# liuyuan-pal/Gen6D

Hardware: NVIDIA H100
Metric: poses/sec end-to-end (128^2 crop, 64 refs, 3 refine iters) (higher is better)
Workload: dtype f32

## Files before the change

### gen6d_b200/_lib.py

```python
import ctypes as C
import os
import re

HERE = os.path.dirname(os.path.abspath(__file__))
LIB_PATH = os.path.join(HERE, 'libgen6d_b200.so')
HEADER_PATH = os.path.join(os.path.dirname(HERE), 'include', 'gen6d_b200.h')

G6D_DET_MAX_SCALES = 8
G6D_GLUE_MAX_OBJECTS = 16
G6D_DET_MAX_INSTANCES = 16
G6D_DET_MAX_PEAK_RADIUS = 3
G6D_ATTENTION_MAX_SMEM_FLOATS = 12288 - 32
G6D_FRAMES_MAX = 1024
G6D_FRAME_RGB, G6D_FRAME_NV12 = 0, 1
G6D_DRAW_MAX_BOXES = 16
PRO_NONE, PRO_AFFINE, PRO_AFFINE_RELU, PRO_CORR = 0, 1, 2, 3
ACT_NONE, ACT_RELU, ACT_LEAKY01 = 0, 1, 2
TC_TF32, TC_F16 = 0, 1
TC_PRENORM, TC_REUSE_IM2COL, TC_FOLD_SPLITS = 1, 4, 32


class ConvDesc(C.Structure):
    _fields_ = [(n, C.c_int) for n in ('B', 'D', 'H', 'W', 'Cin', 'in_cstride', 'in_coff', 'Cout', 'kd', 'kh', 'kw',
                                       'stride', 'pd', 'ph', 'pw', 'Do', 'Ho', 'Wo', 'out_cstride', 'out_coff',
                                       'prologue')] + [('group_rows', C.c_longlong), ('act', C.c_int), ('max_chain_k', C.c_int),
                                                      ('plan_rows', C.c_int)]


class DetMaps(C.Structure):
    _fields_ = [('n_scales', C.c_int), ('rfn', C.c_int), ('hs', C.c_int), ('ws', C.c_int),
                ('map', (C.c_void_p * 3) * G6D_DET_MAX_SCALES),
                ('H', (C.c_int * 3) * G6D_DET_MAX_SCALES), ('W', (C.c_int * 3) * G6D_DET_MAX_SCALES),
                ('mu', C.c_float * 3), ('inv_sigma', C.c_float * 3), ('clip', C.c_float)]

# ... 158 lines not shown
```

### gen6d_b200/csrc/conv_tc.cu

```cuda
#include <cuda_fp16.h>
#include <string.h>

#include "tc_common.cuh"

namespace g6d {

constexpr int TC_BM = 128;
constexpr int TC_PRODUCER_WARPS = 8;
constexpr int TC_CONSUMER_WARPS = 8;
constexpr int TC_THREADS = (TC_PRODUCER_WARPS + TC_CONSUMER_WARPS) * 32;
constexpr int TC_ISSUER = TC_PRODUCER_WARPS * 32;
constexpr int TC_PRODUCER_REGS = 96, TC_CONSUMER_REGS = 160;
static_assert(TC_PRODUCER_WARPS * TC_PRODUCER_REGS + TC_CONSUMER_WARPS * TC_CONSUMER_REGS <= 65536 / 32, "register file of one SM");
constexpr int TC_FOLD_PRODUCER_REGS = 40, TC_FOLD_CONSUMER_REGS = 216;
static_assert(TC_PRODUCER_WARPS * TC_FOLD_PRODUCER_REGS + TC_CONSUMER_WARPS * TC_FOLD_CONSUMER_REGS <= 65536 / 32, "register file of one SM");
static_assert(TC_BM == 64 * (TC_CONSUMER_WARPS / 4), "one 64-row wgmma tile per consumer warpgroup");
constexpr int TC_MAX_K_PER_CHAIN = 2048;

template <int KIND> struct KindCfg;
template <> struct KindCfg<G6D_TC_TF32> {
    static constexpr int BK = 32;
    static constexpr int NV = 1;
    static constexpr float CROSS = 1.f;
};
template <> struct KindCfg<G6D_TC_F16> {
    static constexpr int BK = 64;
    static constexpr int NV = 2;
    static constexpr float CROSS = 1.f / 2048.f;
};
constexpr float F16_LO_SCALE = 2048.f;
constexpr int TC2_RING = 2, FLAT_RING = 3;
// ... 234 lines not shown
                                              int lane) {
    sum_chains<BN, KIND>(acc, cross, n_acc);
    store_tile<BN>(cross, dst0, dst1, n_base, Cout, bias, act, partial, vec2, stats, group, lane);
}

constexpr int TC2_PF_BYTES = 12 * 128;

template <int BN> struct Tc2Cfg {
    static constexpr int A_BYTES = TC_BM * 128;
    static constexpr int B_BYTES = BN * 128;
    static constexpr int STAGE_BYTES = 2 * A_BYTES + 2 * B_BYTES;
    static constexpr int STAGES = (208 * 1024) / STAGE_BYTES > 6 ? 6 : (208 * 1024) / STAGE_BYTES;
    static constexpr int SMEM_BYTES = STAGES * STAGE_BYTES + 1024 + 256;
};

template <int BN> struct Tc2XrCfg {
    static constexpr int BOX_ROWS = 144;
    static constexpr int BOX_BYTES = BOX_ROWS * 128;
    static constexpr int BOXES = 3;
    static constexpr int B_BYTES = BN * 128;
    static constexpr int B_STAGES = 6;
    static constexpr int SMEM_BYTES = BOXES * 2 * BOX_BYTES + B_STAGES * 2 * B_BYTES + 1024 + 256;
};
static_assert(Tc2XrCfg<64>::SMEM_BYTES <= 227 * 1024, "x-reuse rings of BN 64");

struct Tc2Work { int m_tiles, n_tiles, total; };

template <int BN, int KIND, bool FOLD, bool XR>
__global__ void __launch_bounds__(TC_THREADS, 1)
conv_tc2_kernel(const ConvTcP p, const Tc2Work wk, const __grid_constant__ CUtensorMap map_hi,
                const __grid_constant__ CUtensorMap map_lo, const __grid_constant__ CUtensorMap map_a) {
    using Cfg = Tc2Cfg<BN>;
    using XC = Tc2XrCfg<BN>;
    using KC = KindCfg<KIND>;
    constexpr int NPW = TC_PRODUCER_WARPS;
    constexpr int STAGES = Cfg::STAGES;
    constexpr int NMAIN = AccCfg<BN>::NMAIN;
    constexpr int BK = KC::BK, NV = KC::NV;
    constexpr int RSTEP = NPW * 4;
    constexpr int ROWS = TC_BM / RSTEP;
    constexpr int RING = TC2_RING;
    constexpr int PF = TC2_PF_BYTES / 128;
    extern __shared__ uint8_t smem_raw[];
    const uint32_t base = (smem_u32(smem_raw) + 1023u) & ~1023u;
    const uint32_t bar_base = base + STAGES * Cfg::STAGE_BYTES;
    auto a_hi = [&](int s) { return base + s * Cfg::STAGE_BYTES; };
    auto a_lo = [&](int s) { return base + s * Cfg::STAGE_BYTES + Cfg::A_BYTES; };
    auto b_hi = [&](int s) { return base + s * Cfg::STAGE_BYTES + 2 * Cfg::A_BYTES; };
    auto b_lo = [&](int s) { return base + s * Cfg::STAGE_BYTES + 2 * Cfg::A_BYTES + Cfg::B_BYTES; };
    auto full_a = [&](int s) { return bar_base + 8 * s; };
// ... 2 lines not shown
    auto box_hi = [&](int s) { return base + s * 2 * XC::BOX_BYTES; };
    auto box_lo = [&](int s) { return base + s * 2 * XC::BOX_BYTES + XC::BOX_BYTES; };
    const uint32_t xb_base = base + XC::BOXES * 2 * XC::BOX_BYTES;
    auto xb_hi = [&](int s) { return xb_base + s * 2 * XC::B_BYTES; };
    auto xb_lo = [&](int s) { return xb_base + s * 2 * XC::B_BYTES + XC::B_BYTES; };
    const uint32_t xbar = xb_base + XC::B_STAGES * 2 * XC::B_BYTES;
    auto box_full = [&](int s) { return xbar + 8 * s; };
    auto box_empty = [&](int s) { return xbar + 8 * (XC::BOXES + s); };
    auto xb_full = [&](int s) { return xbar + 8 * (2 * XC::BOXES + s); };
    auto xb_empty = [&](int s) { return xbar + 8 * (2 * XC::BOXES + XC::B_STAGES + s); };

    const int warp = threadIdx.x >> 5, lane = threadIdx.x & 31;
    if (XR && threadIdx.x == TC_ISSUER) {
        for (int s = 0; s < XC::BOXES; ++s) {
            mbar_init(box_full(s), 1);
            mbar_init(box_empty(s), TC_CONSUMER_WARPS);
        }
        for (int s = 0; s < XC::B_STAGES; ++s) {
            mbar_init(xb_full(s), 1);
            mbar_init(xb_empty(s), TC_CONSUMER_WARPS);
        }
        fence_barrier_init();
        asm volatile("prefetch.tensormap [%0];" ::"l"(&map_hi) : "memory");
        asm volatile("prefetch.tensormap [%0];" ::"l"(&map_lo) : "memory");
        asm volatile("prefetch.tensormap [%0];" ::"l"(&map_a) : "memory");
    } else if (threadIdx.x == TC_ISSUER) {
        for (int s = 0; s < STAGES; ++s) {
            mbar_init(full_a(s), p.split_in ? 1 : NPW);
            mbar_init(full_b(s), 1);
            mbar_init(empty(s), TC_CONSUMER_WARPS);
        }
        fence_barrier_init();
        asm volatile("prefetch.tensormap [%0];" ::"l"(&map_hi) : "memory");
        asm volatile("prefetch.tensormap [%0];" ::"l"(&map_lo) : "memory");
        if (p.split_in) asm volatile("prefetch.tensormap [%0];" ::"l"(&map_a) : "memory");
    }
    __syncthreads();

    auto decode = [&](int w, int& mt, int& nt, int& sp) {
        nt = w % wk.n_tiles; w /= wk.n_tiles;
        mt = w % wk.m_tiles;
        sp = w / wk.m_tiles;
    };
    auto kblocks_of = [&](int sp) { return min(p.kblocks, sp * p.kb_per_split + p.kb_per_split) - sp * p.kb_per_split; };
    const int chains = FOLD ? p.splits : 1;
    auto chain_of = [&](int j, int& mt, int& nt, int& sp) {
        const int w = blockIdx.x + (j / chains) * gridDim.x;
        if (w >= wk.total) return false;
        decode(w, mt, nt, sp);
        sp += j % chains;
        return true;
    };

    if (warp < NPW) {
        setmaxnreg_dec<FOLD ? TC_FOLD_PRODUCER_REGS : TC_PRODUCER_REGS>();
        if (XR && threadIdx.x == 0) {
            const bool vol = p.D > 1 || p.kd > 1;
            const uint32_t box_tx = 2u * p.xr_rows * 128u;
            int g = 0, gb = 0;
            int mt, nt, sp;
            for (int j = 0; chain_of(j, mt, nt, sp); ++j) {
                const int nkb = kblocks_of(sp);
                int m = mt * TC_BM;
                const int xo = m % p.Wp; m /= p.Wp;
                const int yo = m % p.Ho; m /= p.Ho;
                const int zo = m % p.Do;
                const int b = m / p.Do;
                KbIter pf, k;
                pf.start(p, sp, 0);
                k = pf;
                auto prefetch = [&]() {
                    const int kc = pf.tap(p) * p.Cin + pf.cb * BK;
                    tma_prefetch_2d(&map_hi, kc, nt * BN);
                    tma_prefetch_2d(&map_lo, kc, nt * BN);
                    pf.next(p);
                };
#pragma unroll 1
                for (int i = 0; i < min(nkb, PF - 1); ++i) prefetch();
// ... 10 lines not shown
                        } else {
                            tma_im2col_4d(box_hi(s), &map_a, box_full(s), 2 * BK * k.cb, xo - p.pw, yo - p.ph, b, 0, oy);
                            tma_im2col_4d(box_lo(s), &map_a, box_full(s), 2 * BK * k.cb + BK, xo - p.pw, yo - p.ph, b, 0, oy);
                        }
                        ++gb;
                    }
                    const int s = g % XC::B_STAGES;
                    mbar_wait(xb_empty(s), ((g / XC::B_STAGES) & 1) ^ 1, 1, g);
                    mbar_expect_tx(xb_full(s), 2 * XC::B_BYTES);
                    tma_load_2d(xb_hi(s), &map_hi, xb_full(s), k.tap(p) * p.Cin + k.cb * BK, nt * BN);
                    tma_load_2d(xb_lo(s), &map_lo, xb_full(s), k.tap(p) * p.Cin + k.cb * BK, nt * BN);
                }
            }
            return;
        }
        if (XR || FOLD || p.split_in) {
            if (!XR && threadIdx.x == 0) {
                const bool vol = p.D > 1 || p.kd > 1;
                int g = 0;
                int mt, nt, sp;
                for (int j = 0; chain_of(j, mt, nt, sp); ++j) {
                    const int nkb = kblocks_of(sp);
                    int m = mt * TC_BM;
                    const int xo = m % p.Wo; m /= p.Wo;
                    const int yo = m % p.Ho; m /= p.Ho;
                    const int zo = m % p.Do;
                    const int b = m / p.Do;
                    KbIter pf, k;
                    pf.start(p, sp, 0);
                    k = pf;
                    auto prefetch = [&]() {
                        const int kc = pf.tap(p) * p.Cin + pf.cb * BK;
                        tma_prefetch_2d(&map_hi, kc, nt * BN);
                        tma_prefetch_2d(&map_lo, kc, nt * BN);
                        pf.next(p);
                    };
#pragma unroll 1
                    for (int i = 0; i < min(nkb, PF - 1); ++i) prefetch();
// ... 213 lines not shown
            }
            wgmma_wait<0>();
            if (nkb > 0) release(g - 1);
            }

            sum_chains<BN, KIND>(acc, cross, nkb < NMAIN ? nkb : NMAIN);
            if constexpr (FOLD) {
#pragma unroll
                for (int jj = 0; jj < BN / 2; ++jj) run[jj] = (sp == 0 ? 0.f : run[jj]) + cross[jj];
                if (sp < p.splits - 1) continue;
#pragma unroll
                for (int jj = 0; jj < BN / 2; ++jj) cross[jj] = run[jj];
            }
            const bool partial = p.splits > 1 && !FOLD;
            const int n_base = nt * BN;
            const int m0 = mt * TC_BM + 16 * cw + (lane >> 2), m1 = m0 + 8;
            float* out = partial ? p.ws + (long long)sp * p.M * p.Cout + n_base : p.y + p.oco + n_base;
            const long long ld = partial ? p.Cout : p.ocs;
            const bool vec2 = partial ? (p.Cout & 1) == 0
                                      : ((p.ocs & 1) == 0 && (p.oco & 1) == 0 && (reinterpret_cast<uintptr_t>(p.y) & 7) == 0);
            auto dst = [&](int m) -> float* {
                if constexpr (XR) {
                    if (m >= p.Mp) return nullptr;
                    const int q = m / p.Wp, xp = m - q * p.Wp;
                    return xp < p.Wo ? out + ((long long)q * p.Wo + xp) * ld : nullptr;
                } else {
                    return m < p.M ? out + m * ld : nullptr;
                }
            };
            store_tile<BN>(cross, dst(m0), dst(m1), n_base, p.Cout, p.bias,
                           p.act, partial, vec2, p.stats, (long long)(mt * TC_BM + 16 * cw) / p.stats_rows, lane);
        }
    }
}


__global__ void conv_tc_reduce_kernel(const float* __restrict__ ws, const float* __restrict__ bias,
                                      float* __restrict__ y, int M, int Cout, int splits, int ocs, int oco, int act) {
    const long long i = (long long)blockIdx.x * blockDim.x + threadIdx.x;
    if (i >= (long long)M * Cout) return;
    const int n = (int)(i % Cout);
    const long long m = i / Cout;
    float v = 0.f;
    for (int s = 0; s < splits; ++s) v += ws[(long long)s * M * Cout + i];
    if (bias) v += bias[n];
    y[m * ocs + oco + n] = tc_act(v, act);
}

// ... 221 lines not shown
        splits = (int)(kNumSMs / ctas);
        splits = splits > p.kblocks / min_kb ? p.kblocks / min_kb : splits;
        splits = splits < 1 ? 1 : splits;
    }
    const int nmain = tc_nmain(bn);
    const int chain = d->max_chain_k > 0 ? d->max_chain_k * nmain : (K > TC_MAX_K_PER_CHAIN ? TC_MAX_K_PER_CHAIN * nmain : 0);
    const int max_kb = chain > bk ? chain / bk : 1;
    const int min_splits = chain > 0 ? (p.kblocks + max_kb - 1) / max_kb : 1;
    splits = splits < min_splits ? min_splits : splits;
    splits = splits > 64 ? 64 : splits;
    p.kb_per_split = (p.kblocks + splits - 1) / splits;
    p.splits = (p.kblocks + p.kb_per_split - 1) / p.kb_per_split;
    return G6D_OK;
}

template <int BN, int KIND, bool FOLD, bool XR>
static int launch_tc2(const ConvTcP& p, const CUtensorMap& mh, const CUtensorMap& ml, const CUtensorMap& ma, cudaStream_t st) {
    constexpr int SMEM = XR ? Tc2XrCfg<BN>::SMEM_BYTES : Tc2Cfg<BN>::SMEM_BYTES;
    static bool configured = false;
    if (!configured) {
        cudaError_t e = cudaFuncSetAttribute(conv_tc2_kernel<BN, KIND, FOLD, XR>, cudaFuncAttributeMaxDynamicSharedMemorySize, SMEM);
        if (e != cudaSuccess) { set_error("g6d_conv_tc: cannot opt in to %d B of shared memory: %s", SMEM, cudaGetErrorString(e)); return G6D_ECUDA; }
        configured = true;
    }
    Tc2Work wk;
    wk.m_tiles = ceil_div(XR ? p.Mp : p.M, TC_BM); wk.n_tiles = ceil_div(p.Cout, BN);
    const long long total = (long long)wk.m_tiles * wk.n_tiles * (FOLD ? 1 : p.splits);
    wk.total = (int)total;
    const int grid = total < kNumSMs ? (int)total : kNumSMs;
    conv_tc2_kernel<BN, KIND, FOLD, XR><<<grid, TC_THREADS, SMEM, st>>>(p, wk, mh, ml, ma);
    G6D_CHECK_LAUNCH("g6d_conv_tc");
    return G6D_OK;
}

__global__ void split_tf32_kernel(const float* __restrict__ in, float* __restrict__ hi, float* __restrict__ lo, long long n) {
    const long long i = (long long)blockIdx.x * blockDim.x + threadIdx.x;
    if (i >= n) return;
    const float v = in[i];
    const float h = to_tf32(v);
    hi[i] = h;
    lo[i] = to_tf32(v - h);
}
__device__ __forceinline__ void split_f16_scalar(float v, __half& h, __half& l) {
    uint32_t hh, ll;
    split_f16x2(v, 0.f, hh, ll);
// ... 358 lines not shown
    if (!configured) {
        cudaError_t e = cudaFuncSetAttribute(conv_tcflat_kernel<BN, KIND>, cudaFuncAttributeMaxDynamicSharedMemorySize, 227 * 1024);
        if (e != cudaSuccess) { set_error("g6d_conv_tc(flat): cannot opt in to shared memory: %s", cudaGetErrorString(e)); return G6D_ECUDA; }
        configured = true;
    }
    dim3 grid((unsigned)((long long)p.B * p.Do * p.tiles_per_plane), ceil_div(p.Cout, BN), p.splits);
    conv_tcflat_kernel<BN, KIND><<<grid, TC_THREADS, smem, st>>>(p, mh, ml);
    G6D_CHECK_LAUNCH("g6d_conv_tc(flat)");
    return G6D_OK;
}

struct ConvPlan {
    ConvTcP tc;
    ConvFlatP flat;
    bool use_flat;
    int bn, splits, flat_smem;
    long long split_in_off;
    long long ws_bytes;
};

constexpr double TC_FOLD_SLACK = 0.15;

static bool fold_ok(const ConvPlan& pl) {
    if (pl.use_flat || !pl.tc.split_in || pl.splits < 2) return false;
    const long long T = (long long)ceil_div(pl.tc.M, TC_BM) * ceil_div(pl.tc.Cout, pl.bn), S = pl.splits;
    return (double)(ceil_div(T, kNumSMs) * S) <= (1.0 + TC_FOLD_SLACK) * (double)ceil_div(T * S, kNumSMs);
}

static bool split_input_ok(const g6d_conv_desc* d, int kind, int flags, bool use_flat) {
    if (use_flat || kind != G6D_TC_F16 || (d->prologue != G6D_PRO_NONE && !(flags & G6D_TC_PRENORM)) || d->stride != 1 ||
        d->kd * d->kh * d->kw == 1)
        return false;
    if (!split_input_rank5(d)) return d->kw <= 64 && d->kh <= 64 && d->pw < 64 && d->ph < 64;
    auto corners_ok = [](int k, int pad) { return k <= 16 && pad <= 16 && pad - (k - 1) >= -16 && pad - (k - 1) <= 15; };
    return (flags & G6D_TC_REUSE_IM2COL) && corners_ok(d->kw, d->pw) && corners_ok(d->kh, d->ph) && corners_ok(d->kd, d->pd);
}

static bool xr_ok(const g6d_conv_desc* d, const ConvPlan& pl) {
    if (!pl.tc.split_in || !pl.tc.reuse_order || pl.bn != 64 || d->kw < 2 || d->kw > 17) return false;
    if (split_input_rank5(d) && d->pw > 15) return false;
    return (long long)pl.tc.M / pl.tc.Wo * (pl.tc.Wo + d->kw - 1) < (1ll << 31);
}

static int make_plan(const g6d_conv_desc* d, int kind, int flags, ConvPlan& pl) {
    G6D_REQUIRE((flags & ~(G6D_TC_PRENORM | G6D_TC_REUSE_IM2COL | G6D_TC_FOLD_SPLITS)) == 0, "g6d_conv_tc: bad flags %d", flags);
    const int rc = fill_tc_params(d, kind, pl.tc);
    if (rc != G6D_OK) return rc;
    pl.use_flat = fill_flat_params(d, kind, pl.flat, &pl.flat_smem);
    pl.tc.reuse_order = 0;
    if (pl.use_flat && (flags & G6D_TC_REUSE_IM2COL) && split_input_ok(d, kind, flags, false)) {
        pl.use_flat = false;
        pl.tc.reuse_order = 1;
        pl.tc.kb_per_split = pl.flat.cb_per_split * d->kd * d->kh * d->kw;
        pl.tc.splits = pl.flat.splits;
    }
    pl.bn = tc_block_n(d->Cout);
    pl.splits = pl.use_flat ? pl.flat.splits : pl.tc.splits;
    pl.tc.split_in = split_input_ok(d, kind, flags, pl.use_flat) ? 1 : 0;
    pl.tc.fold = (flags & G6D_TC_FOLD_SPLITS) && fold_ok(pl) ? 1 : 0;
    pl.tc.xr = xr_ok(d, pl) ? 1 : 0;
    if (pl.tc.xr) {
        pl.tc.Wp = pl.tc.Wo + d->kw - 1;
        pl.tc.Mp = (int)((long long)pl.tc.M / pl.tc.Wo * pl.tc.Wp);
        pl.tc.xr_rows = (TC_BM + d->kw - 1 + 7) / 8 * 8;
    }
    const long long partials =
        pl.splits > 1 && !pl.tc.fold ? (long long)pl.splits * pl.tc.M * pl.tc.Cout * (long long)sizeof(float) : 0;
    pl.split_in_off = (partials + 255) / 256 * 256;
    pl.ws_bytes = pl.tc.split_in
                      ? pl.split_in_off + (long long)d->B * d->D * d->H * d->W * d->Cin * 2 * (long long)sizeof(__half)
                      : partials;
    return G6D_OK;
}

static bool stats_ok(const ConvPlan& pl, long long stats_rows) {
    if (stats_rows <= 0 || stats_rows % 32 != 0 || pl.tc.M % stats_rows != 0) return false;
    return !(pl.use_flat || pl.tc.reuse_order) || stats_rows % ((long long)pl.flat.Ho * pl.flat.Wo) == 0;
}

template <class P>
static void bind_tensors(P& p, const float* x, const float* bias, const float* ps, const float* pb, float* y, void* ws,
                         double* stats, long long stats_rows) {
    p.x = x; p.bias = bias; p.ps = ps; p.pb = pb; p.y = y; p.ws = static_cast<float*>(ws);
    p.stats = stats; p.stats_rows = stats ? stats_rows : 1;
}

template <int BN, int KIND>
static int launch_plan(const ConvPlan& pl, const CUtensorMap& mh, const CUtensorMap& ml, const CUtensorMap& ma, cudaStream_t st) {
    if (pl.use_flat) return launch_flat<BN, KIND>(pl.flat, pl.flat_smem, mh, ml, st);
    if constexpr (KIND == G6D_TC_F16) {
        if constexpr (BN == 64)
            if (pl.tc.xr) return pl.tc.fold ? launch_tc2<BN, KIND, true, true>(pl.tc, mh, ml, ma, st)
                                            : launch_tc2<BN, KIND, false, true>(pl.tc, mh, ml, ma, st);
        if (pl.tc.fold) return launch_tc2<BN, KIND, true, false>(pl.tc, mh, ml, ma, st);
    }
    return launch_tc2<BN, KIND, false, false>(pl.tc, mh, ml, ma, st);
}
template <int KIND>
static int dispatch(const ConvPlan& pl, const CUtensorMap& mh, const CUtensorMap& ml, const CUtensorMap& ma, cudaStream_t st) {
    if (pl.bn == 128) return launch_plan<128, KIND>(pl, mh, ml, ma, st);
    if (pl.bn == 64) return launch_plan<64, KIND>(pl, mh, ml, ma, st);
    return launch_plan<32, KIND>(pl, mh, ml, ma, st);
}

}
// ... 36 lines not shown
    ConvPlan pl{};
    const int rc = make_plan(desc, kind, flags, pl);
    if (rc != G6D_OK) return rc;
    out4[0] = pl.use_flat ? 1 : 0;
    out4[1] = pl.bn;
    out4[2] = pl.splits;
    out4[3] = pl.tc.split_in;
    return G6D_OK;
}

extern "C" int g6d_conv_tc_plan_v2(const g6d_conv_desc* desc, int kind, int flags, int* out, int n) {
    G6D_REQUIRE(out != nullptr && n > 0, "g6d_conv_tc_plan_v2: null output");
    ConvPlan pl{};
    const int rc = make_plan(desc, kind, flags, pl);
    if (rc != G6D_OK) return rc;
    const int v[6] = {pl.use_flat ? 1 : 0, pl.bn, pl.splits, pl.tc.split_in, pl.tc.fold, pl.tc.xr};
    for (int i = 0; i < n && i < 6; ++i) out[i] = v[i];
    return G6D_OK;
}

extern "C" int g6d_conv_tc_plan(const g6d_conv_desc* desc, int kind, int* out4) {
    return g6d_conv_tc_plan_ex(desc, kind, 0, out4);
}

extern "C" int g6d_conv_tc_ex(const g6d_conv_desc* desc, const float* x, const void* w_hi, const void* w_lo, int w_rows,
                              int kind, const float* bias, const float* pro_scale, const float* pro_shift, float* y,
                              void* ws, double* stats, long long stats_rows, int flags, g6d_stream_t stream) {
    ConvPlan pl{};
    int rc = make_plan(desc, kind, flags, pl);
    if (rc != G6D_OK) return rc;
    const ConvTcP& p = pl.tc;
    if (stats) G6D_REQUIRE(stats_ok(pl, stats_rows), "g6d_conv_tc: fused statistics need groups of whole 32-row slices / planes (stats_rows %lld)", stats_rows);
// ... 126 lines not shown
```

### gen6d_b200/network/backbone.py

```python
import torch

from .. import ops
from .params import VGG11_BLOCKS

BN_EPS = 1e-5


def pack_vgg(params):
    packed = {}
    f = params.features
    with torch.no_grad():
        for block in VGG11_BLOCKS:
            for slot in block:
                conv, bn = f[slot], f[slot + 1]
                scale = (bn.weight / torch.sqrt(bn.running_var + BN_EPS)).float().contiguous()
                bias = ((conv.bias - bn.running_mean) * scale + bn.bias).float().contiguous()
                packed[slot] = ops.pack_conv(conv.weight, stride=1, pad=1, cout_scale=scale, bias_override=bias)
    return packed


def vgg_pyramid(packed, x, full_res=False):
    outs = []
    fused = not full_res and x.shape[1] % 2 == 0 and x.shape[2] % 2 == 0 and x.shape[3] == 4
    for bi, block in enumerate(VGG11_BLOCKS):
        if bi == 0 and fused:
            outs.append(None)
            x = ops.vgg_first_block(x, packed[block[0]])
            continue
        if bi > 0 and not (bi == 1 and fused):
            x = ops.maxpool2x2(x)
        for slot in block:
            x = ops.conv(x, packed[slot], act=ops.ACT_NONE if slot == 25 else ops.ACT_RELU, reuse_im2col=True,
                         fold_splits=True)
        outs.append(x)
    outs.append(ops.maxpool2x2(x))
    return outs


def vgg_v1(packed, x):
    p = vgg_pyramid(packed, x)
    return p[3], p[4], p[5]


def vgg_v3(packed, x):
    p = vgg_pyramid(packed, x)
    return p[2], p[3], p[4]
```

### gen6d_b200/network/detector.py

```python
from dataclasses import dataclass

import numpy as np
import torch

from .. import ops
from .backbone import pack_vgg, vgg_v1
from .base import Branches, PackedModule
from .params import VGG11BNParams, detector_heads


@dataclass
class DetectorRefs:
    center_feats: list
    kernels: list
    shape: tuple = (120, 120)

    @property
    def rfn(self):
        return self.center_feats[0].shape[0]


class Detector(PackedModule):
    default_cfg = {
        'vgg_score_stats': [[36.264317, 13.151907], [13910.291, 5345.965], [829.70807, 387.98788]],
# ... 64 lines not shown
    def scale_sizes(self, hq, wq):
        out = []
        for s in self.cfg['detection_scales']:
            ht, wt = int(np.round(hq * 2 ** s)), int(np.round(wq * 2 ** s))
            if ht % 32 != 0:
                ht = (ht // 32 + 1) * 32
            if wt % 32 != 0:
                wt = (wt // 32 + 1) * 32
            out.append((ht, wt))
        return out

    def _raw_correlation(self, que01):
        feats = self._features(que01)
        out = []
        for f, pc in zip(feats, self.ref_kernels):
            y = ops.conv(f, pc, reuse_im2col=True, fold_splits=True)
            rows = getattr(pc, 'rows', None)
            out.append(ops.det_corr_rowsum(y, *rows) if rows is not None else y)
        return out

    def _raw_correlation_objects(self, que01, kernels, n_obj, rfn):
        feats = self._features(que01)
        out = []
        for f, pc in zip(feats, kernels):
            y = ops.conv(f, pc, reuse_im2col=True, fold_splits=True)
            k = pc.rows[0] if pc.rows is not None else 1
            m = ops.det_corr_rowsum_objects(y, n_obj, k, rfn)
            out.append(m.reshape(n_obj * m.shape[1], *m.shape[2:]))
        return out

    def _detect_nhwc(self, que01, return_taps=False):
        if self.ref_kernels is None:
            raise RuntimeError('Detector: load_ref_imgs / load_impl must be called first')
        return self._detect_maps(que01, self._raw_correlation, que01.shape[0], self.refs.rfn, return_taps)

    def _detect_objects_nhwc(self, que01, kernels, n_obj, rfn, return_taps=False):
        return self._detect_maps(que01, lambda cur: self._raw_correlation_objects(cur, kernels, n_obj, rfn),
                                 n_obj * que01.shape[0], rfn, return_taps)

    def _detect_maps(self, que01, correlate, rows, rfn, return_taps):
# ... 7 lines not shown
            cur = que01 if (ht, wt) == (hq, wq) else ops.resize_bilinear(que01, ht, wt)
            return correlate(cur)

        maps = [br.run(i, lambda ht=ht, wt=wt: one_scale(ht, wt)) for i, (ht, wt) in enumerate(scales)]
        br.join()
        sizes = [[(r.shape[1], r.shape[2]) for r in raw] for raw in maps]
        feats = ops.det_score_fuse(maps, sizes, rfn, hs, ws, self.cfg['vgg_score_stats'], self.cfg['vgg_score_max'],
                                   p['w1'], p['b1'], p['w2'], p['b2'], rows)
        outs = {}
        heads = ('score_predict', 'scale_predict', 'offset_predict')
        hb = Branches(len(heads))

        def one_head(head):
            x = feats
            for i, pc in enumerate(p[head]):
                x = ops.conv(x, pc, act=ops.ACT_RELU if i < 2 else ops.ACT_NONE, reuse_im2col=True, fold_splits=True)
            return x

        for i, head in enumerate(heads):
            outs[head] = hb.run(i, lambda head=head: one_head(head))
        hb.join()
        if return_taps:
            outs['raw'] = maps
            outs['scores_feats'] = feats
        return outs

    def _detect_u8(self, u8):
        o = self._detect_nhwc(ops.preprocess_u8(u8, out_c=3, imagenet_norm=False))
        out, _ = ops.det_parse(o['score_predict'], o['scale_predict'], o['offset_predict'], self.pool_ratio)
        return out

# ... 35 lines not shown
```

### gen6d_b200/network/refiner.py

```python
import threading
from dataclasses import dataclass, field

import numpy as np
import torch

from .. import ops
from .backbone import pack_vgg, vgg_v3
from .base import Branches, PackedModule, linear_as_conv
from .params import RefineFeatureParams, RefineRegressorParams, RefineVolumeParams

IN_EPS = 1e-5
_UPLOAD_LOCK = threading.Lock()
IM2COL = dict(prenorm=True, reuse_im2col=True, fold_splits=True)


@dataclass
class RefinerRefs:
    database: object
    ids: list
    dev: dict = field(default_factory=dict)
    src: dict = field(default_factory=dict)


class VolumeRefiner(PackedModule):
    default_cfg = {'refiner_sample_num': 32}

    def __init__(self, cfg):
        self.cfg = {**self.default_cfg, **cfg}
# ... 208 lines not shown
```

### gen6d_b200/network/selector.py

```python
from dataclasses import dataclass

import numpy as np
import torch

from .. import ops
from .backbone import pack_vgg, vgg_v1
from .base import Branches, PackedModule, linear_as_conv
from .params import SEL_TOWER_POST, SEL_TOWERS, VGG11BNParams, selector_modules

IN_EPS = 1e-5


class LocalComm:
    rank, world, capturable = 0, 1, True

    def all_reduce_sum(self, t):
        return t

    def all_gather_cat(self, t, dim=0):
        return t

    def shard_range(self, n):
        return 0, n

# ... 114 lines not shown

    def _s2_counters(self):
        n = 3 * self.ref_shape[0] * self.ref_shape[1]
        c = self.__dict__.get('_s2_done')
        if c is None or c.numel() != n or c.device != self.device:
            c = torch.zeros(n, device=self.device, dtype=torch.int32)
            self.__dict__['_s2_done'] = c
        return c

    def _finalize(self, ws, rows_total):
        return ops.instnorm_finalize(self.comm.all_reduce_sum(ws), rows_total, IN_EPS)

    def _tower_conv(self, level, i, st, Q, S, cat_buf):
        pc, post = self.packed()['towers'][level][i]
        x = st['x']
        kw = dict(prenorm=True, reuse_im2col=True, fold_splits=True)
        if i == 0:
            rows = x.shape[0] * x.shape[1] * x.shape[2]
            y = torch.empty(Q * x.shape[0], x.shape[1], x.shape[2], pc.cout, device=x.device, dtype=torch.float32)
            ws = [ops.conv(x, pc, prologue=ops.PRO_CORR, pro_scale=st['ps'][q], pro_shift=st['pb'][q], group_rows=S,
                           out=y[q * S:(q + 1) * S], stats_rows=rows, **kw)[1] for q in range(Q)]
            return y, (ws[0] if Q == 1 else torch.cat(ws, 0)), rows
        rows = x.shape[0] * x.shape[1] * x.shape[2] // Q
        if i + 1 == len(self.packed()['towers'][level]):
            ops.conv(x, pc, prologue=st['pro'], pro_scale=st['ps'], pro_shift=st['pb'], group_rows=S, out=cat_buf,
                     out_coff=256 * level, plan_rows=rows, **kw)
            return None
        return ops.conv(x, pc, prologue=st['pro'], pro_scale=st['ps'], pro_shift=st['pb'], group_rows=S, stats_rows=rows,
                        plan_rows=rows, **kw) + (rows,)

    @staticmethod
# ... 221 lines not shown
```

### gen6d_b200/ops.py

```python
import ctypes as C
import os
from dataclasses import dataclass
from typing import Optional

import torch

from . import _lib
from ._lib import ACT_LEAKY01, ACT_NONE, ACT_RELU, PRO_AFFINE, PRO_AFFINE_RELU, PRO_CORR, PRO_NONE


WARP_JOB_BYTES = 88


def _stream():
    return C.c_void_p(torch.cuda.current_stream().cuda_stream)


def _p(t, dtype=torch.float32):
    if t is None:
        return None
    if not (t.is_cuda and t.dtype == dtype and t.is_contiguous()):
        raise ValueError(f'expected a contiguous CUDA {dtype} tensor, got {t.dtype} {t.device} '
                         f'contiguous={t.is_contiguous()} shape={tuple(t.shape)}')
    return C.c_void_p(t.data_ptr())
# ... 556 lines not shown
    hi = torch.empty(x.shape, device=x.device, dtype=_tc_dtype(kind))
    lo = torch.empty_like(hi)
    _call('g6d_split_operand', _p(x), _p(hi, hi.dtype), _p(lo, lo.dtype), x.numel(), kind, _stream())
    return hi, lo, kind


def transpose_to_packed(x2d):
    rows, cols = x2d.shape
    out = torch.empty(cols, (rows + 3) // 4 * 4, device=x2d.device, dtype=torch.float32)
    _call('g6d_transpose2d', _p(x2d), _p(out), rows, cols, _stream())
    return out


def conv(x, pc, prologue=PRO_NONE, pro_scale=None, pro_shift=None, group_rows=1, act=ACT_NONE,
         in_coff=0, out=None, out_coff=0, stats_rows=None, prenorm=False, reuse_im2col=False, fold_splits=False,
         plan_rows=0):
    four = x.dim() == 4
    if four:
        B, H, W, cs = x.shape
        D = 1
    else:
        B, D, H, W, cs = x.shape
    kd, kh, kw = pc.k
    pd, ph, pw = pc.pad
    s = pc.stride
    Do, Ho, Wo = (D + 2 * pd - kd) // s + 1, (H + 2 * ph - kh) // s + 1, (W + 2 * pw - kw) // s + 1
    if out is None:
        shape = (B, Ho, Wo, pc.cout) if four else (B, Do, Ho, Wo, pc.cout)
        out = torch.empty(shape, device=x.device, dtype=torch.float32)
    d = _lib.ConvDesc(B=B, D=D, H=H, W=W, Cin=pc.cin, in_cstride=cs, in_coff=in_coff, Cout=pc.cout, kd=kd, kh=kh,
                      kw=kw, stride=s, pd=pd, ph=ph, pw=pw, Do=Do, Ho=Ho, Wo=Wo, out_cstride=out.shape[-1],
                      out_coff=out_coff, prologue=prologue, group_rows=group_rows, act=act, max_chain_k=pc.max_chain_k,
                      plan_rows=plan_rows)
    work = 2.0 * B * Do * Ho * Wo * pc.cout * kd * kh * kw * pc.cin
    M = B * Do * Ho * Wo
    stats = None
    if pc.w_hi is not None and conv_path() == 'tc' and _lib.lib().g6d_conv_tc_supported(C.byref(d), pc.kind):
        flags = ((_lib.TC_PRENORM if prenorm else 0) | (_lib.TC_REUSE_IM2COL if reuse_im2col else 0)
                 | (_lib.TC_FOLD_SPLITS if fold_splits else 0))
        nbytes = _lib.lib().g6d_conv_tc_workspace_bytes_ex(C.byref(d), pc.kind, flags)
        if nbytes < 0:
            _lib.check(-1, 'g6d_conv_tc_workspace_bytes_ex')
        ws = torch.empty(nbytes // 4, device=x.device, dtype=torch.float32) if nbytes > 0 else None
        fuse = stats_rows is not None and _lib.lib().g6d_conv_tc_stats_supported(C.byref(d), pc.kind, stats_rows)
        if fuse:
            stats = torch.empty(M // stats_rows, pc.cout, 2, device=x.device, dtype=torch.float64)
        def tag(d=d, kind=pc.kind, flags=flags):
            plan = (C.c_int * 6)()
            _lib.check(_lib.lib().g6d_conv_tc_plan_v2(C.byref(d), kind, flags, plan, 6), 'g6d_conv_tc_plan_v2')
            a_op = (' prenorm' if prologue != PRO_NONE else ' im2col') if plan[3] else ''
            if flags & _lib.TC_REUSE_IM2COL and plan[3]:
                plain = (C.c_int * 4)()
                _lib.check(_lib.lib().g6d_conv_tc_plan_ex(C.byref(d), kind, flags & ~_lib.TC_REUSE_IM2COL, plain),
                           'g6d_conv_tc_plan_ex')
                a_op += '-ro' if plain[0] else ''
            a_op += '-xr' if plan[5] else ''
            return (f'M={M} N={pc.cout} K={kd * kh * kw * pc.cin} k={kd}x{kh}x{kw} s={s} pro={prologue} '
                    f'{"reuse" if plan[0] else "persist"} BN={plan[1]} splits={plan[2]}{" fold" if plan[4] else ""}{a_op}')
        _call('g6d_conv_tc_ex', C.byref(d), _p(x), _p(pc.w_hi, pc.w_hi.dtype), _p(pc.w_lo, pc.w_lo.dtype), pc.w_hi.shape[0],
              pc.kind, _p(pc.bias), _p(pro_scale), _p(pro_shift), _p(out), _p(ws), _p(stats, torch.float64), stats_rows or 0,
              flags, _stream(), work=work, tag=tag, key='g6d_conv_tc')
    else:
        if pc.w is None:
            raise _lib.Gen6DLibraryError('this operand was packed for the tensor-core path only and the problem is not supported there')
        nbytes = _lib.lib().g6d_conv_workspace_bytes(C.byref(d))
        if nbytes < 0:
            _lib.check(-1, 'g6d_conv_workspace_bytes')
        ws = torch.empty(nbytes // 4, device=x.device, dtype=torch.float32) if nbytes > 0 else None
        _call('g6d_conv', C.byref(d), _p(x), _p(pc.w), _p(pc.bias), _p(pro_scale), _p(pro_shift), _p(out), _p(ws), _stream(),
              work=work)
    if stats_rows is None:
# ... 166 lines not shown
```

### include/gen6d_b200.h

```cpp
#ifndef GEN6D_B200_H
#define GEN6D_B200_H

#include <stdint.h>

#ifdef __cplusplus
extern "C" {
#endif

#define G6D_OK 0
#define G6D_EINVAL (-1)
#define G6D_ECUDA (-2)

typedef void* g6d_stream_t;

const char* g6d_last_error(void);
int g6d_version(void);
long long g6d_launch_count(void);

int g6d_preprocess_u8(const uint8_t* img, float* out, long long n_pixels, int out_c, int imagenet_norm,
                      g6d_stream_t stream);
typedef struct g6d_warp_job {
    const uint8_t* src;
    int rows, cols;
    double M[9];
// ... 225 lines not shown
                         const float* cout_scale, g6d_stream_t stream);
#define G6D_TC_TF32 0
#define G6D_TC_F16 1
int g6d_conv_tc_supported(const g6d_conv_desc* desc, int kind);
int g6d_debug_desc_shift(float* out, int shift, int mode, g6d_stream_t stream);
int g6d_conv_tc_debug(int* host_out8);
long long g6d_conv_tc_workspace_bytes(const g6d_conv_desc* desc, int kind);
int g6d_conv_tc_stats_supported(const g6d_conv_desc* desc, int kind, long long stats_rows);
int g6d_conv_tc_plan(const g6d_conv_desc* desc, int kind, int* out4);
int g6d_conv_tc(const g6d_conv_desc* desc, const float* x, const void* w_hi, const void* w_lo, int w_rows, int kind,
                const float* bias, const float* pro_scale, const float* pro_shift, float* y, void* ws,
                double* stats, long long stats_rows, g6d_stream_t stream);
#define G6D_TC_PRENORM 1
#define G6D_TC_REUSE_IM2COL 4
#define G6D_TC_FOLD_SPLITS 32
int g6d_conv_tc_plan_ex(const g6d_conv_desc* desc, int kind, int flags, int* out4);
int g6d_conv_tc_plan_v2(const g6d_conv_desc* desc, int kind, int flags, int* out, int n);
long long g6d_conv_tc_workspace_bytes_ex(const g6d_conv_desc* desc, int kind, int flags);
int g6d_conv_tc_ex(const g6d_conv_desc* desc, const float* x, const void* w_hi, const void* w_lo, int w_rows, int kind,
                   const float* bias, const float* pro_scale, const float* pro_shift, float* y, void* ws,
                   double* stats, long long stats_rows, int flags, g6d_stream_t stream);
int g6d_pack_conv_weight_tc(const float* w, void* out_hi, void* out_lo, int Cout, int Cin, int Cin_pad, int taps,
                            int rows_pad, const float* cout_scale, int kind, g6d_stream_t stream);
int g6d_split_operand(const float* in, void* hi, void* lo, long long n, int kind, g6d_stream_t stream);
int g6d_transpose2d(const float* in, float* out, int rows, int cols, g6d_stream_t stream);
int g6d_linear_smallm(const float* x, const float* w, const float* bias, float* y, int M, int N, int K, int act,
                      g6d_stream_t stream);

#define G6D_DET_MAX_SCALES 8
typedef struct g6d_det_maps {
// ... 59 lines not shown
```

Baseline: 132.0.

## Add 192-row tall tile variant for x-reuse F16 conv kernel

Adds a tall-tile path for the x-reuse implicit-GEMM conv kernel. It uses 192-row M tiles with 4 producer and 12 consumer warps, shrinks producer registers and resizes the shared box ring to 2 boxes of 208 rows. A cost heuristic enables it only when the wave count with 192-row tiles, scaled by 1.35, does not exceed the 128-row wave count. The aim is fewer tiles and waves for large-M convs and better reuse of weight tiles. The trade-off is fewer producer warps and a shallower activation ring, which could stall the consumers. All network call sites now pass tall=True.

Measured after the change: 132.6, median of 6. No clear change (+0.4%).

```diff
diff --git a/gen6d_b200/_lib.py b/gen6d_b200/_lib.py
--- a/gen6d_b200/_lib.py
+++ b/gen6d_b200/_lib.py
@@ -17,7 +17,7 @@
 PRO_NONE, PRO_AFFINE, PRO_AFFINE_RELU, PRO_CORR = 0, 1, 2, 3
 ACT_NONE, ACT_RELU, ACT_LEAKY01 = 0, 1, 2
 TC_TF32, TC_F16 = 0, 1
-TC_PRENORM, TC_REUSE_IM2COL, TC_FOLD_SPLITS = 1, 4, 32
+TC_PRENORM, TC_REUSE_IM2COL, TC_FOLD_SPLITS, TC_TALL = 1, 4, 32, 128
 
 
 class ConvDesc(C.Structure):
diff --git a/gen6d_b200/csrc/conv_tc.cu b/gen6d_b200/csrc/conv_tc.cu
--- a/gen6d_b200/csrc/conv_tc.cu
+++ b/gen6d_b200/csrc/conv_tc.cu
@@ -15,6 +15,13 @@
 constexpr int TC_FOLD_PRODUCER_REGS = 40, TC_FOLD_CONSUMER_REGS = 216;
 static_assert(TC_PRODUCER_WARPS * TC_FOLD_PRODUCER_REGS + TC_CONSUMER_WARPS * TC_FOLD_CONSUMER_REGS <= 65536 / 32, "register file of one SM");
 static_assert(TC_BM == 64 * (TC_CONSUMER_WARPS / 4), "one 64-row wgmma tile per consumer warpgroup");
+constexpr int TC_TALL_BM = 192;
+constexpr int TC_TALL_PRODUCER_WARPS = 4, TC_TALL_CONSUMER_WARPS = 12;
+constexpr int TC_TALL_PRODUCER_REGS = 24;
+static_assert((TC_TALL_PRODUCER_WARPS + TC_TALL_CONSUMER_WARPS) * 32 == TC_THREADS, "the same block size as 128-row tiles");
+static_assert(TC_TALL_BM == 64 * (TC_TALL_CONSUMER_WARPS / 4), "one 64-row wgmma tile per consumer warpgroup");
+static_assert(TC_TALL_PRODUCER_WARPS * TC_TALL_PRODUCER_REGS + TC_TALL_CONSUMER_WARPS * TC_CONSUMER_REGS <= 65536 / 32,
+              "register file of one SM");
 constexpr int TC_MAX_K_PER_CHAIN = 2048;
 
 template <int KIND> struct KindCfg;
@@ -279,26 +286,29 @@
     static constexpr int SMEM_BYTES = STAGES * STAGE_BYTES + 1024 + 256;
 };
 
-template <int BN> struct Tc2XrCfg {
-    static constexpr int BOX_ROWS = 144;
+template <int BN, bool TALL> struct Tc2XrCfg {
+    static constexpr int BOX_ROWS = TALL ? 208 : 144;
     static constexpr int BOX_BYTES = BOX_ROWS * 128;
-    static constexpr int BOXES = 3;
+    static constexpr int BOXES = TALL ? 2 : 3;
     static constexpr int B_BYTES = BN * 128;
     static constexpr int B_STAGES = 6;
     static constexpr int SMEM_BYTES = BOXES * 2 * BOX_BYTES + B_STAGES * 2 * B_BYTES + 1024 + 256;
 };
-static_assert(Tc2XrCfg<64>::SMEM_BYTES <= 227 * 1024, "x-reuse rings of BN 64");
+static_assert(Tc2XrCfg<64, false>::SMEM_BYTES <= 227 * 1024, "x-reuse rings of BN 64");
+static_assert(Tc2XrCfg<64, true>::SMEM_BYTES <= 227 * 1024, "x-reuse rings of BN 64, tall tiles");
 
 struct Tc2Work { int m_tiles, n_tiles, total; };
 
-template <int BN, int KIND, bool FOLD, bool XR>
-__global__ void __launch_bounds__(TC_THREADS, 1)
-conv_tc2_kernel(const ConvTcP p, const Tc2Work wk, const __grid_constant__ CUtensorMap map_hi,
-                const __grid_constant__ CUtensorMap map_lo, const __grid_constant__ CUtensorMap map_a) {
+template <int BN, int KIND, bool FOLD, bool XR, bool TALL>
+__device__ __forceinline__ void conv_tc2_body(const ConvTcP& p, const Tc2Work& wk, const CUtensorMap& map_hi,
+                                              const CUtensorMap& map_lo, const CUtensorMap& map_a) {
+    static_assert(!TALL || (XR && !FOLD), "tall tiles: x reuse, and a folded CTA's consumers need more registers");
+    constexpr int BM = TALL ? TC_TALL_BM : TC_BM;
     using Cfg = Tc2Cfg<BN>;
-    using XC = Tc2XrCfg<BN>;
+    using XC = Tc2XrCfg<BN, TALL>;
     using KC = KindCfg<KIND>;
-    constexpr int NPW = TC_PRODUCER_WARPS;
+    constexpr int NPW = TALL ? TC_TALL_PRODUCER_WARPS : TC_PRODUCER_WARPS;
+    constexpr int NCW = TALL ? TC_TALL_CONSUMER_WARPS : TC_CONSUMER_WARPS;
     constexpr int STAGES = Cfg::STAGES;
     constexpr int NMAIN = AccCfg<BN>::NMAIN;
     constexpr int BK = KC::BK, NV = KC::NV;
@@ -331,11 +341,11 @@
     if (XR && threadIdx.x == TC_ISSUER) {
         for (int s = 0; s < XC::BOXES; ++s) {
             mbar_init(box_full(s), 1);
-            mbar_init(box_empty(s), TC_CONSUMER_WARPS);
+            mbar_init(box_empty(s), NCW);
         }
         for (int s = 0; s < XC::B_STAGES; ++s) {
             mbar_init(xb_full(s), 1);
-            mbar_init(xb_empty(s), TC_CONSUMER_WARPS);
+            mbar_init(xb_empty(s), NCW);
         }
         fence_barrier_init();
         asm volatile("prefetch.tensormap [%0];" ::"l"(&map_hi) : "memory");
@@ -345,7 +355,7 @@
         for (int s = 0; s < STAGES; ++s) {
             mbar_init(full_a(s), p.split_in ? 1 : NPW);
             mbar_init(full_b(s), 1);
-            mbar_init(empty(s), TC_CONSUMER_WARPS);
+            mbar_init(empty(s), NCW);
         }
         fence_barrier_init();
         asm volatile("prefetch.tensormap [%0];" ::"l"(&map_hi) : "memory");
@@ -370,7 +380,7 @@
     };
 
     if (warp < NPW) {
-        setmaxnreg_dec<FOLD ? TC_FOLD_PRODUCER_REGS : TC_PRODUCER_REGS>();
+        setmaxnreg_dec<TALL ? TC_TALL_PRODUCER_REGS : (FOLD ? TC_FOLD_PRODUCER_REGS : TC_PRODUCER_REGS)>();
         if (XR && threadIdx.x == 0) {
             const bool vol = p.D > 1 || p.kd > 1;
             const uint32_t box_tx = 2u * p.xr_rows * 128u;
@@ -378,7 +388,7 @@
             int mt, nt, sp;
             for (int j = 0; chain_of(j, mt, nt, sp); ++j) {
                 const int nkb = kblocks_of(sp);
-                int m = mt * TC_BM;
+                int m = mt * BM;
                 const int xo = m % p.Wp; m /= p.Wp;
                 const int yo = m % p.Ho; m /= p.Ho;
                 const int zo = m % p.Do;
@@ -419,14 +429,14 @@
             }
             return;
         }
-        if (XR || FOLD || p.split_in) {
+        if (TALL || XR || FOLD || p.split_in) {
             if (!XR && threadIdx.x == 0) {
                 const bool vol = p.D > 1 || p.kd > 1;
                 int g = 0;
                 int mt, nt, sp;
                 for (int j = 0; chain_of(j, mt, nt, sp); ++j) {
                     const int nkb = kblocks_of(sp);
-                    int m = mt * TC_BM;
+                    int m = mt * BM;
                     const int xo = m % p.Wo; m /= p.Wo;
                     const int yo = m % p.Ho; m /= p.Ho;
                     const int zo = m % p.Do;
@@ -670,7 +680,7 @@
             }
             const bool partial = p.splits > 1 && !FOLD;
             const int n_base = nt * BN;
-            const int m0 = mt * TC_BM + 16 * cw + (lane >> 2), m1 = m0 + 8;
+            const int m0 = mt * BM + 16 * cw + (lane >> 2), m1 = m0 + 8;
             float* out = partial ? p.ws + (long long)sp * p.M * p.Cout + n_base : p.y + p.oco + n_base;
             const long long ld = partial ? p.Cout : p.ocs;
             const bool vec2 = partial ? (p.Cout & 1) == 0
@@ -685,9 +695,23 @@
                 }
             };
             store_tile<BN>(cross, dst(m0), dst(m1), n_base, p.Cout, p.bias,
-                           p.act, partial, vec2, p.stats, (long long)(mt * TC_BM + 16 * cw) / p.stats_rows, lane);
-        }
-    }
+                           p.act, partial, vec2, p.stats, (long long)(mt * BM + 16 * cw) / p.stats_rows, lane);
+        }
+    }
+}
+
+template <int BN, int KIND, bool FOLD, bool XR>
+__global__ void __launch_bounds__(TC_THREADS, 1)
+conv_tc2_kernel(const ConvTcP p, const Tc2Work wk, const __grid_constant__ CUtensorMap map_hi,
+                const __grid_constant__ CUtensorMap map_lo, const __grid_constant__ CUtensorMap map_a) {
+    conv_tc2_body<BN, KIND, FOLD, XR, false>(p, wk, map_hi, map_lo, map_a);
+}
+
+template <int BN, int KIND>
+__global__ void __launch_bounds__(TC_THREADS, 1)
+conv_tc2_tall_kernel(const ConvTcP p, const Tc2Work wk, const __grid_constant__ CUtensorMap map_hi,
+                     const __grid_constant__ CUtensorMap map_lo, const __grid_constant__ CUtensorMap map_a) {
+    conv_tc2_body<BN, KIND, false, true, true>(p, wk, map_hi, map_lo, map_a);
 }
 
 
@@ -939,21 +963,24 @@
     return G6D_OK;
 }
 
-template <int BN, int KIND, bool FOLD, bool XR>
+template <int BN, int KIND, bool FOLD, bool XR, bool TALL = false>
 static int launch_tc2(const ConvTcP& p, const CUtensorMap& mh, const CUtensorMap& ml, const CUtensorMap& ma, cudaStream_t st) {
-    constexpr int SMEM = XR ? Tc2XrCfg<BN>::SMEM_BYTES : Tc2Cfg<BN>::SMEM_BYTES;
+    constexpr int BM = TALL ? TC_TALL_BM : TC_BM;
+    constexpr int SMEM = XR ? Tc2XrCfg<BN, TALL>::SMEM_BYTES : Tc2Cfg<BN>::SMEM_BYTES;
+    auto kernel = conv_tc2_kernel<BN, KIND, FOLD, XR>;
+    if constexpr (TALL) kernel = conv_tc2_tall_kernel<BN, KIND>;
     static bool configured = false;
     if (!configured) {
-        cudaError_t e = cudaFuncSetAttribute(conv_tc2_kernel<BN, KIND, FOLD, XR>, cudaFuncAttributeMaxDynamicSharedMemorySize, SMEM);
+        cudaError_t e = cudaFuncSetAttribute(kernel, cudaFuncAttributeMaxDynamicSharedMemorySize, SMEM);
         if (e != cudaSuccess) { set_error("g6d_conv_tc: cannot opt in to %d B of shared memory: %s", SMEM, cudaGetErrorString(e)); return G6D_ECUDA; }
         configured = true;
     }
     Tc2Work wk;
-    wk.m_tiles = ceil_div(XR ? p.Mp : p.M, TC_BM); wk.n_tiles = ceil_div(p.Cout, BN);
+    wk.m_tiles = ceil_div(XR ? p.Mp : p.M, BM); wk.n_tiles = ceil_div(p.Cout, BN);
     const long long total = (long long)wk.m_tiles * wk.n_tiles * (FOLD ? 1 : p.splits);
     wk.total = (int)total;
     const int grid = total < kNumSMs ? (int)total : kNumSMs;
-    conv_tc2_kernel<BN, KIND, FOLD, XR><<<grid, TC_THREADS, SMEM, st>>>(p, wk, mh, ml, ma);
+    kernel<<<grid, TC_THREADS, SMEM, st>>>(p, wk, mh, ml, ma);
     G6D_CHECK_LAUNCH("g6d_conv_tc");
     return G6D_OK;
 }
@@ -1342,6 +1369,7 @@
     ConvTcP tc;
     ConvFlatP flat;
     bool use_flat;
+    bool tall;
     int bn, splits, flat_smem;
     long long split_in_off;
     long long ws_bytes;
@@ -1370,8 +1398,20 @@
     return (long long)pl.tc.M / pl.tc.Wo * (pl.tc.Wo + d->kw - 1) < (1ll << 31);
 }
 
+constexpr double TC_TALL_COST = 1.35;
+
+static bool tall_ok(const ConvPlan& pl, int flags) {
+    if (!(flags & G6D_TC_TALL) || !pl.tc.xr || pl.tc.fold) return false;
+    const long long rows = pl.tc.Mp;
+    const long long items = (long long)ceil_div(pl.tc.Cout, pl.bn) * pl.splits;
+    const long long r128 = ceil_div(ceil_div(rows, (long long)TC_BM) * items, (long long)kNumSMs);
+    const long long r192 = ceil_div(ceil_div(rows, (long long)TC_TALL_BM) * items, (long long)kNumSMs);
+    return TC_TALL_COST * (double)r192 <= (double)r128;
+}
+
 static int make_plan(const g6d_conv_desc* d, int kind, int flags, ConvPlan& pl) {
-    G6D_REQUIRE((flags & ~(G6D_TC_PRENORM | G6D_TC_REUSE_IM2COL | G6D_TC_FOLD_SPLITS)) == 0, "g6d_conv_tc: bad flags %d", flags);
+    G6D_REQUIRE((flags & ~(G6D_TC_PRENORM | G6D_TC_REUSE_IM2COL | G6D_TC_FOLD_SPLITS | G6D_TC_TALL)) == 0,
+                "g6d_conv_tc: bad flags %d", flags);
     const int rc = fill_tc_params(d, kind, pl.tc);
     if (rc != G6D_OK) return rc;
     pl.use_flat = fill_flat_params(d, kind, pl.flat, &pl.flat_smem);
@@ -1390,8 +1430,9 @@
     if (pl.tc.xr) {
         pl.tc.Wp = pl.tc.Wo + d->kw - 1;
         pl.tc.Mp = (int)((long long)pl.tc.M / pl.tc.Wo * pl.tc.Wp);
-        pl.tc.xr_rows = (TC_BM + d->kw - 1 + 7) / 8 * 8;
-    }
+    }
+    pl.tall = tall_ok(pl, flags);
+    if (pl.tc.xr) pl.tc.xr_rows = ((pl.tall ? TC_TALL_BM : TC_BM) + d->kw - 1 + 7) / 8 * 8;
     const long long partials =
         pl.splits > 1 && !pl.tc.fold ? (long long)pl.splits * pl.tc.M * pl.tc.Cout * (long long)sizeof(float) : 0;
     pl.split_in_off = (partials + 255) / 256 * 256;
@@ -1417,6 +1458,8 @@
 static int launch_plan(const ConvPlan& pl, const CUtensorMap& mh, const CUtensorMap& ml, const CUtensorMap& ma, cudaStream_t st) {
     if (pl.use_flat) return launch_flat<BN, KIND>(pl.flat, pl.flat_smem, mh, ml, st);
     if constexpr (KIND == G6D_TC_F16) {
+        if constexpr (BN == 64)
+            if (pl.tall) return launch_tc2<BN, KIND, false, true, true>(pl.tc, mh, ml, ma, st);
         if constexpr (BN == 64)
             if (pl.tc.xr) return pl.tc.fold ? launch_tc2<BN, KIND, true, true>(pl.tc, mh, ml, ma, st)
                                             : launch_tc2<BN, KIND, false, true>(pl.tc, mh, ml, ma, st);
@@ -1483,8 +1526,8 @@
     ConvPlan pl{};
     const int rc = make_plan(desc, kind, flags, pl);
     if (rc != G6D_OK) return rc;
-    const int v[6] = {pl.use_flat ? 1 : 0, pl.bn, pl.splits, pl.tc.split_in, pl.tc.fold, pl.tc.xr};
-    for (int i = 0; i < n && i < 6; ++i) out[i] = v[i];
+    const int v[7] = {pl.use_flat ? 1 : 0, pl.bn, pl.splits, pl.tc.split_in, pl.tc.fold, pl.tc.xr, pl.tall ? TC_TALL_BM : TC_BM};
+    for (int i = 0; i < n && i < 7; ++i) out[i] = v[i];
     return G6D_OK;
 }
 
diff --git a/gen6d_b200/network/backbone.py b/gen6d_b200/network/backbone.py
--- a/gen6d_b200/network/backbone.py
+++ b/gen6d_b200/network/backbone.py
@@ -31,7 +31,7 @@
             x = ops.maxpool2x2(x)
         for slot in block:
             x = ops.conv(x, packed[slot], act=ops.ACT_NONE if slot == 25 else ops.ACT_RELU, reuse_im2col=True,
-                         fold_splits=True)
+                         fold_splits=True, tall=True)
         outs.append(x)
     outs.append(ops.maxpool2x2(x))
     return outs
diff --git a/gen6d_b200/network/detector.py b/gen6d_b200/network/detector.py
--- a/gen6d_b200/network/detector.py
+++ b/gen6d_b200/network/detector.py
@@ -102,7 +102,7 @@
         feats = self._features(que01)
         out = []
         for f, pc in zip(feats, self.ref_kernels):
-            y = ops.conv(f, pc, reuse_im2col=True, fold_splits=True)
+            y = ops.conv(f, pc, reuse_im2col=True, fold_splits=True, tall=True)
             rows = getattr(pc, 'rows', None)
             out.append(ops.det_corr_rowsum(y, *rows) if rows is not None else y)
         return out
@@ -111,7 +111,7 @@
         feats = self._features(que01)
         out = []
         for f, pc in zip(feats, kernels):
-            y = ops.conv(f, pc, reuse_im2col=True, fold_splits=True)
+            y = ops.conv(f, pc, reuse_im2col=True, fold_splits=True, tall=True)
             k = pc.rows[0] if pc.rows is not None else 1
             m = ops.det_corr_rowsum_objects(y, n_obj, k, rfn)
             out.append(m.reshape(n_obj * m.shape[1], *m.shape[2:]))
@@ -149,7 +149,7 @@
         def one_head(head):
             x = feats
             for i, pc in enumerate(p[head]):
-                x = ops.conv(x, pc, act=ops.ACT_RELU if i < 2 else ops.ACT_NONE, reuse_im2col=True, fold_splits=True)
+                x = ops.conv(x, pc, act=ops.ACT_RELU if i < 2 else ops.ACT_NONE, reuse_im2col=True, fold_splits=True, tall=True)
             return x
 
         for i, head in enumerate(heads):
diff --git a/gen6d_b200/network/refiner.py b/gen6d_b200/network/refiner.py
--- a/gen6d_b200/network/refiner.py
+++ b/gen6d_b200/network/refiner.py
@@ -11,7 +11,7 @@
 
 IN_EPS = 1e-5
 _UPLOAD_LOCK = threading.Lock()
-IM2COL = dict(prenorm=True, reuse_im2col=True, fold_splits=True)
+IM2COL = dict(prenorm=True, reuse_im2col=True, fold_splits=True, tall=True)
 
 
 @dataclass
diff --git a/gen6d_b200/network/selector.py b/gen6d_b200/network/selector.py
--- a/gen6d_b200/network/selector.py
+++ b/gen6d_b200/network/selector.py
@@ -152,7 +152,7 @@
     def _tower_conv(self, level, i, st, Q, S, cat_buf):
         pc, post = self.packed()['towers'][level][i]
         x = st['x']
-        kw = dict(prenorm=True, reuse_im2col=True, fold_splits=True)
+        kw = dict(prenorm=True, reuse_im2col=True, fold_splits=True, tall=True)
         if i == 0:
             rows = x.shape[0] * x.shape[1] * x.shape[2]
             y = torch.empty(Q * x.shape[0], x.shape[1], x.shape[2], pc.cout, device=x.device, dtype=torch.float32)
diff --git a/gen6d_b200/ops.py b/gen6d_b200/ops.py
--- a/gen6d_b200/ops.py
+++ b/gen6d_b200/ops.py
@@ -594,7 +594,7 @@
 
 def conv(x, pc, prologue=PRO_NONE, pro_scale=None, pro_shift=None, group_rows=1, act=ACT_NONE,
          in_coff=0, out=None, out_coff=0, stats_rows=None, prenorm=False, reuse_im2col=False, fold_splits=False,
-         plan_rows=0):
+         plan_rows=0, tall=False):
     four = x.dim() == 4
     if four:
         B, H, W, cs = x.shape
@@ -617,7 +617,7 @@
     stats = None
     if pc.w_hi is not None and conv_path() == 'tc' and _lib.lib().g6d_conv_tc_supported(C.byref(d), pc.kind):
         flags = ((_lib.TC_PRENORM if prenorm else 0) | (_lib.TC_REUSE_IM2COL if reuse_im2col else 0)
-                 | (_lib.TC_FOLD_SPLITS if fold_splits else 0))
+                 | (_lib.TC_FOLD_SPLITS if fold_splits else 0) | (_lib.TC_TALL if tall else 0))
         nbytes = _lib.lib().g6d_conv_tc_workspace_bytes_ex(C.byref(d), pc.kind, flags)
         if nbytes < 0:
             _lib.check(-1, 'g6d_conv_tc_workspace_bytes_ex')
@@ -626,8 +626,8 @@
         if fuse:
             stats = torch.empty(M // stats_rows, pc.cout, 2, device=x.device, dtype=torch.float64)
         def tag(d=d, kind=pc.kind, flags=flags):
-            plan = (C.c_int * 6)()
-            _lib.check(_lib.lib().g6d_conv_tc_plan_v2(C.byref(d), kind, flags, plan, 6), 'g6d_conv_tc_plan_v2')
+            plan = (C.c_int * 7)()
+            _lib.check(_lib.lib().g6d_conv_tc_plan_v2(C.byref(d), kind, flags, plan, 7), 'g6d_conv_tc_plan_v2')
             a_op = (' prenorm' if prologue != PRO_NONE else ' im2col') if plan[3] else ''
             if flags & _lib.TC_REUSE_IM2COL and plan[3]:
                 plain = (C.c_int * 4)()
@@ -635,6 +635,7 @@
                            'g6d_conv_tc_plan_ex')
                 a_op += '-ro' if plain[0] else ''
             a_op += '-xr' if plan[5] else ''
+            a_op += ' tall' if plan[6] > 128 else ''
             return (f'M={M} N={pc.cout} K={kd * kh * kw * pc.cin} k={kd}x{kh}x{kw} s={s} pro={prologue} '
                     f'{"reuse" if plan[0] else "persist"} BN={plan[1]} splits={plan[2]}{" fold" if plan[4] else ""}{a_op}')
         _call('g6d_conv_tc_ex', C.byref(d), _p(x), _p(pc.w_hi, pc.w_hi.dtype), _p(pc.w_lo, pc.w_lo.dtype), pc.w_hi.shape[0],
diff --git a/include/gen6d_b200.h b/include/gen6d_b200.h
--- a/include/gen6d_b200.h
+++ b/include/gen6d_b200.h
@@ -263,6 +263,7 @@
 #define G6D_TC_PRENORM 1
 #define G6D_TC_REUSE_IM2COL 4
 #define G6D_TC_FOLD_SPLITS 32
+#define G6D_TC_TALL 128
 int g6d_conv_tc_plan_ex(const g6d_conv_desc* desc, int kind, int flags, int* out4);
 int g6d_conv_tc_plan_v2(const g6d_conv_desc* desc, int kind, int flags, int* out, int n);
 long long g6d_conv_tc_workspace_bytes_ex(const g6d_conv_desc* desc, int kind, int flags);
```
